# m-hamza-mughal/RAG-Gesture

Measured on AMD Instinct MI355X. Metric: SMPL-X frames/sec, len150 DDIM-50 + insertion guidance; 1/2/4/8 GPU, higher is better.
Workload: dtype bf16

## Files before the change

include/rg_gesture.h:

```cpp
#ifndef RG_GESTURE_H
#define RG_GESTURE_H

#include <stdint.h>

#ifdef __cplusplus
extern "C" {
#endif

typedef struct rg_handle rg_handle;

enum rg_status {
  RG_OK = 0,
  RG_ERR_INVALID = -1,
  RG_ERR_HIP = -2,
  RG_ERR_NO_DEVICE = -3
};

#define RG_VERSION 124
int rg_version(void);
int rg_create(rg_handle** out, int device);
void rg_destroy(rg_handle* h);
const char* rg_last_error(rg_handle* h);
int rg_num_cus(rg_handle* h);

int rg_ddim_update(rg_handle* h, const float* x, const float* x0, float* x_out, int64_t n,
                   float c_recip, float c_recipm1, float c_a, float c_b, void* stream);

int rg_cfg_ddim_update(rg_handle* h, const float* out, const float* x, float* x_out, float* x0_out,
                       const float* js, int B, int T, int D, float w_c, float w_u,
                       float c_recip, float c_recipm1, float c_a, float c_b, void* stream);
int rg_cfg_ddim_update_rows(rg_handle* h, const float* out_cond, const float* out_uncond, const float* x, float* x_out,
                            float* x_out2, const float* js, int B, int T, int D, float w_c, float w_u,
                            float c_recip, float c_recipm1, float c_a, float c_b, void* stream);

int rg_cfg_ddpm_update(rg_handle* h, const float* out, const float* x, const float* noise, float* x_out,
                       const float* js, int B, int T, int D, float w_c, float w_u, float c1, float c2, float sigma,
                       void* stream);

typedef struct rg_glue_args {
  const float* out_c_a;
  const float* out_u_a;
  float* x_a;
  const float* out_c_b;
  const float* out_u_b;
  float* x_b;
  float* x_b_copy;
  const float* in_seq_next;
  const float* noise_next;
  const float* js;
  int n_a, n_b, T, D;
  int g_iter_next;
// ... 139 lines not shown
#define RG_SEQ_U_FF2_0 12
#define RG_SEQ_U_FF1_1 13
#define RG_SEQ_U_FF2_1 14
#define RG_SEQ_U_FFO 15
typedef struct rg_seq_args {
  const void* wstream;
  const void* pstream;
  const void* ustream;
  const void* afrag;
  const float* x;
  const float* tbias;
  const float* src_mask;
  const float* qmask;
  float* head;
  float* dump;
  float* xbuf;
  void* gbuf;
  const int* form;
  int L, B, T, S;
  int step, step_b, split;
  int dump_stage, dump_layer;
  int pairs;
  int twin;
  int* glue_ctr;
  rg_glue_args glue;
} rg_seq_args;

int rg_seq_forward(rg_handle* h, const rg_seq_args* args_host, void* stream);
int rg_seq2_forward(rg_handle* h, const rg_seq_args* args_host, void* stream);

#define RG_SEQ_MANY_MAX 8
int rg_seq_forward_many(rg_handle* h, const rg_seq_args* const* args_host, int n, void* stream);

#define RG_LANE_STRIDE 32
int rg_seqx_forward(rg_handle* h, const rg_seq_args* args_host, void* stream);
int rg_lane_form(rg_handle* h, int* state, int lane, int nlanes, int narrow_wgs, int wide_wgs, int budget, void* stream);

typedef struct rg_venc_args {
  const void* wstream;
  const void* pstream;
  const float* x;
  float* out;
  float* xbuf;
  float* dump;
  int nseq, S, nb, dump_block;
  const int* post_rows;
  float* post_mu;
  float* post_logvar;
  int post_nrows, pad_;
} rg_venc_args;

int rg_venc_forward(rg_handle* h, const rg_venc_args* args_host, void* stream);
int rg_venc_forward_grouped(rg_handle* h, const rg_venc_args* args_host, int n, void* stream);

typedef struct rg_vdec_args {
  const void* wstream;
  const void* pstream;
  float* x;
  const float* pos;
  void* qimg;
  void* kbuf;
  void* vt;
  float* xbuf;
  float* dump;
  int nseq, nb, step, pad_;
  const float* latent;
// ... 419 lines not shown
```

rag-gesture_amd/csrc/rg_seq.hip:

```cpp
#ifndef RG_SEQ_BODY_ONLY
#define RG_PACK2_ONE
#endif
#include "rg_common.h"
#include "rg_stationary.h"
#include "rg_tail.h"
#include "rg_seq_host.h"

namespace {

constexpr int RD = 7;
constexpr int UPL = RG_SEQ_UPL;
constexpr int OFF_P0 = 0;
constexpr int OFF_P1 = TP * 1024;
constexpr int OFF_RING = 2 * TP * 1024;
constexpr int MAX_SEG = 8 * 34 + 5;
constexpr int OFF_DESC = OFF_RING + NW * RD * 1024;
constexpr int OFF_STAT = OFF_DESC + MAX_SEG * 16;
constexpr int LDS_BYTES = OFF_STAT + NW * TP * 2 * 4;
static_assert(LDS_BYTES <= 160 * 1024, "LDS budget");

#define U(name) U_##name = RG_SEQ_U_##name
enum { U(KV), U(KV2), U(Q), U(SAO), U(MIXX), U(Q3_0), U(MIX_0), U(Q3_1), U(MIX_1), U(Q3_2), U(MIX_2), U(FF1_0), U(FF2_0), U(FF1_1), U(FF2_1), U(FFO) };
#undef U
#define SEG(u, k) ((u) << 2 | (k))
// ... 491 lines not shown
  const int npass = pairs ? 2 : 1;
#pragma unroll 1
  for (int pass = 0; pass < npass; ++pass) {
    run_sequence(a, seq0 + pass * B, smem);
    __syncthreads();
    int* const ctr = rg_tail::late_ctr(arg_base);
    if (ctr && !a.dump_stage) {
      const int c = seq0 + pass * B - (seq0 + pass * B >= B ? B : 0);
      rg_tail::arrive_and_glue<NTH>(ctr, c, c, reinterpret_cast<int*>(smem), __builtin_amdgcn_readfirstlane(threadIdx.x >> 6), arg_base);
    }
  }
}

#ifndef RG_SEQ_BODY_ONLY
__global__ void __launch_bounds__(NTH) rg_seq_kernel(const rg_seq_args a) {
  extern __shared__ __attribute__((aligned(16))) unsigned char smem[];
  RG_OWN_THE_SIMD();
  seq_block(a, blockIdx.x, a.pairs, smem);
}

extern "C" int rg_seq_forward(rg_handle* h, const rg_seq_args* args_host, void* stream) {
  const std::string why = rg_seq_refusal(RG_SEQ_ENTRY, args_host);
  if (!why.empty()) { if (h) h->err = why; return RG_ERR_INVALID; }
  const rg_seq_args& a = *args_host;
  static rg_attr_once lds_once;
  RG_RESERVE_LDS(h, lds_once, rg_seq_kernel, LDS_BYTES);
  rg_prof_scope prof(h, stream, 3, rg_seq_flops(a));
  hipLaunchKernelGGL(rg_seq_kernel, dim3(a.pairs ? a.B : 2 * a.B), dim3(NTH), LDS_BYTES, rg_stream(stream), a);
  RG_CHECK_LAUNCH(h);
  prof.stop();
  return RG_OK;
}

struct rg_seq_many_block {
  rg_seq_args a[RG_SEQ_MANY_MAX];
  int end[RG_SEQ_MANY_MAX];
};
static_assert(sizeof(rg_seq_many_block) <= 4096, "the parameter block must fit the kernarg segment");

__global__ void __launch_bounds__(NTH) rg_seq_many_kernel(const rg_seq_many_block p) {
  extern __shared__ __attribute__((aligned(16))) unsigned char smem[];
  RG_OWN_THE_SIMD();
  const int block = blockIdx.x;
  int s = 0, first = 0;
#pragma unroll
  for (int i = 0; i + 1 < RG_SEQ_MANY_MAX; ++i)
    if (block >= p.end[i]) { s = i + 1; first = p.end[i]; }
  s = __builtin_amdgcn_readfirstlane(s);
  seq_block(p.a[s], block - first, 0, smem, (unsigned)(offsetof(rg_seq_many_block, a) + s * sizeof(rg_seq_args)));
}

extern "C" int rg_seq_forward_many(rg_handle* h, const rg_seq_args* const* args_host, int n, void* stream) {
  const std::string why = rg_seq_many_refusal(args_host, n);
  if (!why.empty()) { if (h) h->err = why; return RG_ERR_INVALID; }
  rg_seq_many_block p{};
  int total = 0;
  double flops = 0.0;
  for (int i = 0; i < RG_SEQ_MANY_MAX; ++i) {
    if (i < n) {
      p.a[i] = *args_host[i];
      total += 2 * p.a[i].B;
      flops += rg_seq_flops(p.a[i]);
    }
    p.end[i] = total;
  }
  static rg_attr_once lds_once;
  RG_RESERVE_LDS(h, lds_once, rg_seq_many_kernel, LDS_BYTES);
  rg_prof_scope prof(h, stream, 3, flops);
  hipLaunchKernelGGL(rg_seq_many_kernel, dim3(total), dim3(NTH), LDS_BYTES, rg_stream(stream), p);
  RG_CHECK_LAUNCH(h);
  prof.stop();
// ... 4 lines not shown
```

rag-gesture_amd/csrc/rg_seq2.hip:

```cpp
#if !defined(RG_SEQ_BODY_ONLY) && !defined(RG2_PACK_TWO)
#define RG_PACK2_ONE
#endif
#include "rg_common.h"
#include "rg_stationary.h"
#include "rg_tail.h"
#include "rg_seq_host.h"

namespace {

constexpr int RD = 6;
constexpr int UPL = RG_SEQ_UPL;
constexpr int PANEL = TP * 1024;
constexpr int OFF_RING = 2 * PANEL;
constexpr int NSEG_COND = 36, NSEG_UNC = 19, NSEG_TWIN = 34;
constexpr int NSEG_MAX = NSEG_COND > NSEG_TWIN ? NSEG_COND : NSEG_TWIN;
constexpr int MAX_SEG = 8 * NSEG_MAX + 5;
constexpr int OFF_DESC = OFF_RING + NW * RD * 1024;
constexpr int OFF_STAT = OFF_DESC + ((MAX_SEG * 8 + 15) & ~15);
constexpr int STAT_HALF = 2 * NW * TP * 2;
constexpr int LDS_BYTES = OFF_STAT + 2 * STAT_HALF * 4;
static_assert(LDS_BYTES <= 160 * 1024, "LDS budget");

#define U(name) U_##name = RG_SEQ_U_##name
enum { U(KV), U(KV2), U(Q), U(SAO), U(MIXX), U(Q3_0), U(MIX_0), U(Q3_1), U(MIX_1), U(Q3_2), U(MIX_2), U(FF1_0), U(FF2_0), U(FF1_1), U(FF2_1), U(FFO) };
// ... 925 lines not shown
__global__ void __launch_bounds__(NTH) rg_seq2_kernel(const rg_seq_args a) {
  extern __shared__ __attribute__((aligned(16))) unsigned char smem[];
#ifndef RG2_SHARE_SIMD
  RG_OWN_THE_SIMD();
#endif
  seq2_block(a, blockIdx.x, smem);
}

__global__ void __launch_bounds__(NTH) rg_seq2_twin_kernel(const rg_seq_args a) {
  extern __shared__ __attribute__((aligned(16))) unsigned char smem[];
#ifndef RG2_SHARE_SIMD
  RG_OWN_THE_SIMD();
#endif
  const int clip = blockIdx.x;
  run_pair<true>(a, clip, clip + a.B, smem);
  __syncthreads();
  if (rg_tail::late_ctr() && !a.dump_stage) rg_tail::glue_own<NTH>(clip, __builtin_amdgcn_readfirstlane(threadIdx.x >> 6));
}

extern "C" int rg_seq2_forward(rg_handle* h, const rg_seq_args* args_host, void* stream) {
  const std::string why = rg_seq_refusal(RG_SEQ2_ENTRY, args_host);
  if (!why.empty()) { if (h) h->err = why; return RG_ERR_INVALID; }
  const rg_seq_args& a = *args_host;
  static rg_attr_once lds_once, lds_once_twin;
  if (a.twin) { RG_RESERVE_LDS(h, lds_once_twin, rg_seq2_twin_kernel, LDS_BYTES); }
  else { RG_RESERVE_LDS(h, lds_once, rg_seq2_kernel, LDS_BYTES); }
  rg_prof_scope prof(h, stream, 3, rg_seq_flops(a));
  if (a.twin) hipLaunchKernelGGL(rg_seq2_twin_kernel, dim3(a.B), dim3(NTH), LDS_BYTES, rg_stream(stream), a);
  else hipLaunchKernelGGL(rg_seq2_kernel, dim3(seq2_grid(a.B, a.split, a.pairs)), dim3(NTH), LDS_BYTES, rg_stream(stream), a);
  RG_CHECK_LAUNCH(h);
  prof.stop();
  return RG_OK;
}
#endif
```

rag-gesture_amd/csrc/rg_seq_host.h:

```cpp
#pragma once
#include <string>

#include "../../include/rg_gesture.h"

struct rg_seq_entry { const char *name, *need_bufs, *need_form, *no_dump, *twin_range, *twin_pairs, *no_twin; };
constexpr rg_seq_entry RG_SEQ_ENTRY = {"rg_seq_forward", nullptr, nullptr, nullptr, nullptr, nullptr, nullptr};
constexpr rg_seq_entry RG_SEQ2_ENTRY = {"rg_seq2_forward", "the two-sequence forward needs its scratch buffers xbuf and gbuf", nullptr,
                                        nullptr, "twin must be 0 or 1", "twin and pairs are two launch forms: set one of them", nullptr};
constexpr rg_seq_entry RG_SEQX_ENTRY = {
    "rg_seqx_forward", "the two-sequence form needs its scratch buffers xbuf and gbuf", "form: the lane's flag (rg_lane_form) must be given",
    "diagnostic dumps: use rg_seq_forward / rg_seq2_forward", nullptr, nullptr,
    "the twin form (one clip per workgroup) is not one of the device-chosen forms: use rg_seq2_forward"};

inline bool rg_seq_glue_ok(const rg_seq_args& a) {
  if (!a.glue_ctr) return true;
  const rg_glue_args& g = a.glue;
  if (a.dump_stage || g.n_a < 0 || g.n_b < 0 || g.n_a + g.n_b != a.B || g.T != a.T || g.D != 512 || !g.js || g.g_iter_next < 0) return false;
  if (g.n_a && !(g.out_c_a && g.out_u_a && g.x_a)) return false;
  if (g.n_b && !(g.out_c_b && g.out_u_b && g.x_b)) return false;
  return !g.in_seq_next || g.noise_next;
}

inline std::string rg_seq_refusal(const rg_seq_entry& e, const rg_seq_args* args) {
  const char* why = nullptr;
// ... 6 lines not shown
    else if (e.need_form && !a.form) why = e.need_form;
    else if (!(a.L >= 1 && a.L <= 8 && a.B >= 1 && a.T >= 1 && a.T <= 48)) why = "unsupported shape (T <= 48, L <= 8)";
    else if (!(a.step >= 0 && a.step < a.S && a.step_b >= 0 && a.step_b < a.S)) why = "step out of range";
    else if (e.no_dump && a.dump_stage != 0) why = e.no_dump;
    else if (!e.no_dump && a.dump_stage != 0 && !a.dump) why = "dump_stage needs a dump buffer";
    else if (!(a.pairs == 0 || a.pairs == 1)) why = "pairs must be 0 or 1";
    else if (e.twin_range && !(a.twin == 0 || a.twin == 1)) why = e.twin_range;
    else if (e.twin_pairs && a.twin && a.pairs) why = e.twin_pairs;
    else if (e.no_twin && a.twin) why = e.no_twin;
    else if (!rg_seq_glue_ok(a)) why = "glue_ctr: glue must cover the B clips (n_a + n_b == B, T, D = 512), its pointers set, no dump";
  }
  return why ? std::string(e.name) + ": " + why : std::string();
}

constexpr rg_seq_entry RG_SEQ_MANY_ENTRY = {"rg_seq_forward_many", nullptr, nullptr, "diagnostic dumps: use rg_seq_forward", nullptr, nullptr,
                                            "the twin form is rg_seq2_forward's: a grouped launch runs one workgroup per sequence"};

inline std::string rg_seq_many_refusal(const rg_seq_args* const* args, const int n) {
  const std::string name = std::string(RG_SEQ_MANY_ENTRY.name) + ": ";
  if (!args || n < 1) return name + "null or empty list of sessions";
  if (n > RG_SEQ_MANY_MAX) return name + "too many sessions (at most RG_SEQ_MANY_MAX)";
  for (int i = 0; i < n; ++i) {
    const std::string why = rg_seq_refusal(RG_SEQ_MANY_ENTRY, args[i]);
    if (!why.empty()) return why;
    const rg_seq_args &a = *args[i], &a0 = *args[0];
    if (a.pairs) return name + "pairs is another launch form: a grouped launch runs one workgroup per sequence";
    if (!(a.L == a0.L && a.T == a0.T && a.S == a0.S)) return name + "the sessions must agree in L, T and S";
    if (!(a.wstream == a0.wstream && a.pstream == a0.pstream && a.ustream == a0.ustream))
      return name + "the sessions must share the weight, parameter and table streams";
  }
  return std::string();
}

inline double rg_seq_flops(const rg_seq_args& a) {
  const double unit = 2.0 * a.T * 512 * 512, att = 2.0 * a.T * 32 * 32 * 16;
  const double cond = (RG_SEQ_UPL * a.L + 2) * unit + a.L * (2 + 3) * att, unc = (10 * a.L + 2) * unit + a.L * 2 * att;
  return a.B * (cond + unc);
}
```

rag-gesture_amd/csrc/rg_tail.h:

```cpp
#pragma once
#include "rg_common.h"
#include <cstddef>

namespace rg_tail {

typedef __attribute__((ext_vector_type(4))) float f32x4;
typedef __attribute__((ext_vector_type(4))) unsigned u32x4;
constexpr int COHERENT = 17;

__device__ __forceinline__ float ddim_one(float x, float x0, float c_recip, float c_recipm1, float c_a, float c_b) {
#pragma clang fp contract(off)
  float eps = (c_recip * x - x0) / c_recipm1;
  return x0 * c_a + c_b * eps;
}
__device__ __forceinline__ float cfg_one(float oc, float ou, float jc, float ju, float w_c, float w_u) {
#pragma clang fp contract(off)
  return oc * w_c * jc + ou * w_u * ju;
}

template <typename P>
__device__ __forceinline__ P* uniform_ptr(P* p) {
  const unsigned long long v = reinterpret_cast<unsigned long long>(p);
  return reinterpret_cast<P*>((unsigned long long)__builtin_amdgcn_readfirstlane((unsigned)(v >> 32)) << 32 |
                              (unsigned)__builtin_amdgcn_readfirstlane((unsigned)v));
// ... 143 lines not shown

__device__ __forceinline__ void store_head(float* head, const unsigned byte_offset, const f32x4 v) {
  const auto rs = __builtin_amdgcn_make_buffer_rsrc(head, 0, 0x7fffffff, 0x00020000);
  __builtin_amdgcn_raw_buffer_store_b128(__builtin_bit_cast(u32x4, v), rs, byte_offset, 0, COHERENT);
}

template <int NTH>
__device__ __forceinline__ void arrive_and_glue(int* const ctr, const int c0, const int c1, int* const flag, const int wave,
                                                const unsigned base = 0) {
  const int lane = __builtin_amdgcn_mbcnt_hi(~0u, __builtin_amdgcn_mbcnt_lo(~0u, 0u));
  if (wave == 0 && lane == 0) {
    int m = 0;
    if (__hip_atomic_fetch_add(ctr + c0, 1, __ATOMIC_RELAXED, __HIP_MEMORY_SCOPE_AGENT) & 1) m |= 1;
    if (c1 != c0 && (__hip_atomic_fetch_add(ctr + c1, 1, __ATOMIC_RELAXED, __HIP_MEMORY_SCOPE_AGENT) & 1)) m |= 2;
    *flag = m;
  }
  __syncthreads();
  const int m = *flag;
  __syncthreads();
  if (m == 0) return;
  const rg_glue_args g = late_arg<rg_glue_args>(base + offsetof(rg_seq_args, glue));
  const float ton = two_over_numel(g);
#pragma unroll 1
  for (int q = 0; q < 2; ++q) {
    if (!(m >> q & 1)) continue;
    const int c = q ? c1 : c0;
    const bool ga = c < g.n_a;
    const int cl = ga ? c : c - g.n_a;
    glue_clip<NTH / 64>(g, ga, cl, wave, lane, ton);
  }
}

template <int NTH>
__device__ __forceinline__ void glue_own(const int c, const int wave) {
  const int lane = __builtin_amdgcn_mbcnt_hi(~0u, __builtin_amdgcn_mbcnt_lo(~0u, 0u));
  const rg_glue_args g = late_arg<rg_glue_args>(offsetof(rg_seq_args, glue));
  const bool ga = c < g.n_a;
  glue_clip<NTH / 64>(g, ga, ga ? c : c - g.n_a, wave, lane, two_over_numel(g));
}
}
```

rag-gesture_amd/denoiser.py:

```python
import math

import numpy as np
import torch

from . import capi, gemm as G, seqfwd as SQ

CONDS = ("xf_text", "xf_audio", "xf_spk")
BLOCKS = ("sa_block", "ca_blocks.xf_text", "ca_blocks.xf_audio", "ca_blocks.xf_spk", "ffn")


def _timestep_embedding(timesteps, dim, max_period=10000):
    half = dim // 2
    freqs = torch.exp(-math.log(max_period) * torch.arange(0, half, dtype=torch.float32) / half)
    args = timesteps[:, None].float() * freqs[None]
    return torch.cat([torch.cos(args), torch.sin(args)], dim=-1)


class DenoiserWeights:

    KV_GROUP = 2

    @staticmethod
    def _fold_ln(W, b, gamma, beta, pw, f32):
        Wp = (W.double() * gamma.double()[None, :]).float()
# ... 316 lines not shown
        key = (name, tuple(shape), dtype)
        pool = self.__dict__.setdefault("_scratch_pool", {})
        if key not in pool:
            pool[key] = torch.empty(*shape, device=self.w.dev, dtype=dtype)
        return pool[key]

    def chain_end(self):
        if self.sq is not None:
            self.sq.chain_end()

    def forward(self, x, step, step_b=None, split=None, glue=None):
        w, h, B, R, M, D, T = self.w, self.h, self.B, self.R, self.M, self.w.D, self.w.T
        if split is not None and not (0 < split < B):
            step, step_b, split = (step if split >= B else step_b), None, None
        if self.sq is not None:
            if glue is not None and not x.is_contiguous():
                raise capi.RgError("DenoiserSession.forward(glue=...): x is updated in place and must be contiguous")
            return self.sq.run(x.contiguous(), step, step_b, split, glue=glue)
        if glue is not None:
            raise capi.RgError("DenoiserSession.forward(glue=...): the sequence-stationary engine only")
        if self.ln_mode == "auto":
            out = self._forward_guarded(x, step)
            if split is None:
                return out
        return self._forward_chain(x, step, step_b, split)

    @staticmethod
    def forward_many(sessions, calls):
        for s, kw in zip(sessions, calls):
            if s.sq is None or not kw["x"].is_contiguous():
                raise capi.RgError("DenoiserSession.forward_many: the sequence-stationary engine only, x contiguous")
        return SQ.run_many([s.sq for s in sessions], calls)

    LN_GUARD_SIGMAS = 3.0

    def _forward_guarded(self, x, step):
        if torch.cuda.is_current_stream_capturing():
            raise capi.RgError("DenoiserSession(ln_mode='auto'): run one forward before capturing a graph")
        self._guard = torch.zeros(1, device=self.w.dev)
        self.ln_mode = "folded"
        out = self._forward_chain(x, step)
        self.ln_ratio = float(self._guard.item())
        self._guard = None
        if self.ln_ratio > self.LN_GUARD_SIGMAS ** 2:
            self.ln_mode, self.xa_bf = "prologue", None
            out = self._forward_chain(x, step)
        return out

    def _guard_stats(self, stats):
        if getattr(self, "_guard", None) is not None:
            self.h.call("ln_guard", stats, self.M, stats.shape[1], self.w.D, self._guard)

    def _forward_chain(self, x, step, step_b=None, split=None):
        w, h, B, R, M, D, T = self.w, self.h, self.B, self.R, self.M, self.w.D, self.w.T
        two = split is not None
        if two and (self.abf is None or self.hcat is None):
            raise capi.RgError("two step groups: bf16 launch chain with the stylization pre-pass only")
        xa, xb, xc = self.xa, self.xb, self.xc
        sa_, sb_, sc_ = self.st_a, self.st_b, self.st_c
        sa_w = self.st_a
        G.gemm(h, M=M, N=D, K=D, W=w.w_embed, out=xa, segs=[G.Seg(x.view(B * T, D))], seg_len=D, a_row_mod=B * T,
               bias=w.b_embed, tbias=w.tbias, tb_period=T, stats_out=sa_, out2=self.xa_bf)
        self._guard_stats(sa_)
        for l, lw in enumerate(w.layers):
            ss = w.ss[step, l]
            ssb = w.ss[step_b, l] if two else None
# ... 104 lines not shown
```

rag-gesture_amd/pipeline.py:

```python
import collections
import ctypes
import contextlib
import copy
import os
import time
import types

import torch
import yaml

from . import capi, denoiser, sampler, schedule as sched_mod, seqfwd, vae as vae_mod

MODELS = {}


def register_module(cls):
    MODELS[cls.__name__] = cls
    return cls


def register_with_mmcv(force=False):
    regs = []
    try:
        from mmcv.cnn import MODELS as mmcv_models
# ... 244 lines not shown
        return dict.__iter__(self)

    def copy(self):
        self._ready()
        return dict(dict.items(self))

    __copy__ = copy

    def __deepcopy__(self, memo):
        self._ready()
        return {k: copy.deepcopy(v, memo) for k, v in dict.items(self) if k not in self._PLAIN}

    def __reduce__(self):
        self._ready()
        return (dict, (), None, None, iter([(k, v) for k, v in dict.items(self) if k not in self._PLAIN]))


@register_module
class MotionDiffusion(torch.nn.Module):

    profile_phases = False
    rotation_lanes = None
    form_lanes = None
    _cur_rot = None
    _last_state = None

    def __init__(self, model=None, loss_recon=None, loss_gen=None, loss_contact=None, loss_laplace=None,
                 diffusion_train=None, diffusion_test=None, init_cfg=None, inference_type="ddpm",
                 genloss_acceleration_weight=True, genloss_hands_weight=2, genloss_smooth=True,
                 body_part_lossweights=None, device="cuda", precision="bf16", lanes=2, sample_lanes=None, session_options=None,
                 vae_options=None, async_results=False, slots=2, max_inflight=2, cobatch_lanes="batch", base_lanes=8,
                 batch_lanes=4, lane_streams=None, calibrate_lanes=True, decode_stream=False, dynamic_forms=False, dynamic_budget=None, invert_alone_wide=True, tail_glue=True,
                 cache_exemplar_latents=True, exemplar_cache_bytes=8 << 30, skip_clip_encode=True, grouped_decode=True,
                 grouped_drain=True, **kwargs):
        super().__init__()
        self.grouped_drain = bool(grouped_drain)
        self.grouped_decode = bool(grouped_decode)
        self.cache_exemplar_latents, self.exemplar_cache_bytes = bool(cache_exemplar_latents), int(exemplar_cache_bytes)
        self.skip_clip_encode = bool(skip_clip_encode)
        self.model = build_submodule(model, device=device, **kwargs)
        dt = dict(diffusion_test)
        self.schedule = sched_mod.Schedule(beta_scheduler=dt["beta_scheduler"], diffusion_steps=dt["diffusion_steps"],
                                           respace=dt.get("respace"))
        capi.require(dt.get("model_mean_type", "start_x") == "start_x" and dt.get("classifier_free_guidance_scale", 0) == 0,
                "unsupported argument: requires dt.get(\"model_mean_type\", \"start_x\") == \"start_x\" and dt.get(\"classifier_free_guidance_scale\", 0) == 0")
        self.inference_type = inference_type
        capi.require(inference_type in ("ddim", "ddpm"), "inference_type is 'ddim' (shipped config) or 'ddpm'")
        self.device, self.precision = torch.device(device), precision
        self.training = False
        self.session_options, self.vae_options = dict(session_options or {}), dict(vae_options or {})
        self.vae_options.setdefault("grouped_decode", self.grouped_decode)
        self._state = None
        self._sessions = {}
        self._graphs = {}
        self.use_graphs = True
        self.graph_captures = self.graph_cross_stream_waits = 0
        self._jitter = None
        self.phase_ms = {}
        self.lanes = int(lanes)
        self.base_lanes = max(1, int(base_lanes))
        self.batch_lanes = max(1, int(batch_lanes))
        self.sample_lanes = None if sample_lanes is None else int(sample_lanes)
        self.async_results, self.slots, self.max_inflight = bool(async_results), max(1, int(slots)), max(1, int(max_inflight))
        self.dynamic_forms, self._lane_state = bool(dynamic_forms), None
        self.invert_alone_wide = bool(invert_alone_wide)
        self.tail_glue = bool(tail_glue)
        self.dynamic_budget = None if dynamic_budget is None else int(dynamic_budget)
        self._slot, self._inflight, self._graph_owner, self._slot_done = 0, collections.deque(), {}, {}
# ... 491 lines not shown
            h = self.model.weights.h
            for idx in st.idx_groups:
                h.call("copy_rows", lat.contiguous(), st.in_seq, st.B, 1, st.D, st.T, idx[-1], st.T, idx[0])

    def _take_slot(self, pid, main, lanes, slot=None):
        slot = self._slots[pid] = (self._slots.get(pid, 0) + 1) % self.slots if slot is None else slot
        self._wait_slot(main, lanes, slot)
        self._slot = slot
        return slot

    def _wait_slot(self, main, lanes, slot):
        for lane in dict.fromkeys(lanes):
            for ev in self._slot_done.get((lane, slot), ()):
                main.wait_event(ev)

    @staticmethod
    def _lanes_of(*plans):
        return list(dict.fromkeys(lane for plan in plans for lane, _, _, _ in plan))

    def submit(self, **kwargs):
        if not self.async_results or self.slots < 2:
            raise capi.RgError("submit() needs MotionDiffusion(async_results=True, slots >= 2)")
        self._cob = dict(lane=self._submitted if (self.cobatch_lanes == "batch" and self.batch_lanes > 1) else None)
        self._submitted += 1
        try:
            self.forward(**kwargs)
        finally:
            self._cob = None
        return self._ready.popleft() if self._ready else None

    def flush(self):
        cob, self._cob = self._cob, dict(lane=0)
        try:
            self._finish_pending()
        finally:
            self._cob = cob
        out = list(self._ready)
        self._ready.clear()
        return out

    def _finish_alone(self, st):
        main = st.main = torch.cuda.current_stream()
        st.slot = self._take_slot(st.pid, main, self._lanes_of(st.plan_s))
        for lane, stream, b0, b1 in st.plan_s:
            self._sample_conditions(lane, b0, b1, st.word, st.audio, st.spk, st.motion_mask, st.qmask)
        self._sampling_pass(st)
        return self._tail(st)

    def _pending_upto(self, seq):
        return sorted((p for p in self._pend if self._pend[p].seq <= seq), key=lambda p: self._pend[p].seq)

    def _finish_pending(self, upto=None, resume=None):
        sts = [self._pend.pop(p) for p in self._pending_upto(float("inf") if upto is None else upto)]
        group = self._drain_group(sts) if self.grouped_drain else []
        if group:
            self._drain_grouped(group)
        for st in sts:
            self._ready.append(self._tail(st) if any(st is g for g in group) else self._finish_alone(st))
        if resume is not None:
            self._slot = self._slots[resume.pid] = resume.slot

    DRAIN_SLOT = 0

    def _drain_group(self, sts):
        sett = lambda st: (st.T, st.S, bool(st.use_insertion_guidance), tuple(int(v) for v in st.guidance_iters), float(st.guidance_lr))

        def alone_on_a_lane(st):
            return (st.run_async and st.via_submit and not st.ddpm and st.prev_future is None and st.plan == st.plan_s
                    and len(st.plan_s) == 1 and tuple(st.plan_s[0][2:]) == (0, st.B))
# ... 43 lines not shown
        owners = tuple((st.B, "sample", st.plan_s[0][0], st.slot) for st in order)
        key = ("guided_many" if guided else "sample_many", owners, order[0].T, tuple(st.in_seq is not None for st in order), gi, lr)
        with torch.cuda.stream(g), self._phase("sampling"):
            outs = self._graph_run(key, ins, loop, owner=owners)
            for st, xl in zip(order, outs):
                st.x_out.copy_(xl)

    def _set_conditions_pair(self, sess, key, own, a, b, n_a):
        dev = self.model.weights.dev
        ins = {}
        for tag, (word, audio, spk, mask, qm) in (("a", a), ("b", b)):
            ins["word_" + tag], ins["audio_" + tag] = word.to(dev).float(), audio.to(dev).float()
            ins["spk_" + tag], ins["mask_" + tag] = spk.to(dev).long(), mask.to(dev).float()
            for c in denoiser.CONDS:
                ins["q_%s_%s" % (c, tag)] = qm[c].to(dev).float()

        def run(st):
            for tag, off, fin in (("a", 0, False), ("b", n_a, True)):
                sess.set_conditions(st["word_" + tag], st["audio_" + tag], st["spk_" + tag], st["mask_" + tag],
                                    {c: st["q_%s_%s" % (c, tag)] for c in denoiser.CONDS}, offset=off, finalize=fin)
            return ()
        self._graph_run(key + tuple(tuple(v.shape) for v in ins.values()), ins, run, owner=own)

    def _submit_chain(self, st):
        pend, S, T, D, dev = self._pend.get(st.pid), st.S, st.T, st.D, self.device
        lanes = [(lane, stream, b0, b1, self._exemplars(st, b0, b1)) for lane, stream, b0, b1 in st.plan] if st.use_inversion else []
        so = self.session_options
        groups_ok = self.precision == "bf16" and (self._runs_seq_engine(so) or so.get("styl_prepass", True))
        can_defer = (groups_ok and st.use_inversion and not st.visualize_inversion and not st.ddpm and st.plan == st.plan_s
                     and all(ex for *_, ex in lanes))
        same = pend is not None and can_defer and (pend.B, pend.T) == (st.B, st.T) and \
            [(b0, b1) for _, _, b0, b1 in pend.plan] == [(b0, b1) for _, _, b0, b1 in st.plan]
        if pend is not None and not same:
            self._finish_pending(pend.seq, resume=st)
            pend = None
        if not can_defer:
            self._finish_pending(resume=st)
            for lane, stream, b0, b1 in st.plan_s:
                self._sample_conditions(lane, b0, b1, st.word, st.audio, st.spk, st.motion_mask, st.qmask)
            self._inversion_pass(st)
            self._sampling_pass(st)
            self._ready.append(self._tail(st))
            return None
        if pend is None:
            self._inversion_pass(st)
            for lane, stream, _, _ in st.plan:
                self._slot_done[(lane, st.slot)] = [stream.record_event()]
            self._pend[st.pid] = st
            return None
        main = st.main
        self._fill_prev(pend, main)
        guided = pend.use_insertion_guidance
        gi, lr = tuple(int(v) for v in pend.guidance_iters), float(pend.guidance_lr)
        work = []
        for lane, stream, b0, b1, ex in lanes:
            Bl = b1 - b0
            Ep, cat = self._exemplar_inputs(st, ex, main)
            okey = (Bl + Ep, "cobatch", lane, self._slot)
            sess = self._session(Bl + Ep, "cobatch", lane)
            eqm = exemplar_query_masks(st.qmask, [b for b, _ in ex], Ep)
            self._set_conditions_pair(
                sess, ("cond2", Bl, Ep, lane, self._slot), okey,
                (pend.word[b0:b1], pend.audio[b0:b1], pend.spk[b0:b1], pend.motion_mask[b0:b1], {c: pend.qmask[b0:b1] for c in denoiser.CONDS}),
                (cat("retr_text"), cat("retr_audio"), cat("retr_spkid"), cat("retr_motion_mask"), eqm), Bl)
            work.append((lane, stream, b0, b1, ex, Ep, sess, okey, cat("retr_motion_latent").float().contiguous()))
        for lane, stream, b0, b1, ex, Ep, sess, okey, x_e in work:
            Bl = b1 - b0
            stream.wait_stream(main)
            self._used_on(stream, pend.x, pend.in_seq, pend.inseq_noise, pend.invl, pend.x_out, x_e, st.start_noise, st.invl, st.qmask)
            with torch.cuda.stream(stream):
                sl = lambda t, dim: lane_rows(t, dim, b0, b1)
                ins = dict(xa=sl(pend.x, 0), in_seq=sl(pend.in_seq, 0), noise=sl(pend.inseq_noise, 1),
                           invl=sl(pend.invl, 1) if guided else None, xb=x_e)

                def loop(s, sess=sess, Bl=Bl, Ep=Ep):
                    x_all = torch.cat([s["xa"], s["xb"]], dim=0).contiguous()
                    out_b = torch.empty(S, Ep, T, D, device=dev)
                    sampler.cobatched_loop(sess, x_all, Bl, out_b, inverted_a=s["invl"], guidance_iters=gi, guidance_lr=lr,
                                           inseq_noise_a=s["noise"], in_seq_a=s["in_seq"], tail_glue=self.tail_glue)
                    return x_all[:Bl], out_b
                key = ("cobatch", Bl, Ep, lane, T, self._slot, guided, pend.in_seq is not None, gi, lr, self.tail_glue)
                xl, inv = self._graph_run(key, ins, loop, owner=okey)
                pend.x_out[b0:b1].copy_(xl)
                self._splice(st, ex, inv, Ep)
                self._zero_prev_rows(st, b0, b1)
        pend.main, pend.slot = main, self._slot
        self._ready.append(self._tail(pend))
        self._pend[st.pid] = st
        return None

    def _exemplars(self, st, b0, b1):
        return [(b, q) for b in range(b0, b1) for q in st.retrieval_dict["retr_uncropped_latents"][b].keys()]

    def _exemplar_inputs(self, st, ex, stream):
        dev = self.device
        Ep = bucket(len(ex))
        lat = lambda b, q: st.retrieval_dict["retr_uncropped_latents"][b][q]

        def cat(key):
            parts = [lat(b, q)[key].to(dev) for b, q in ex]
            self._used_on(stream, *parts)
            return pad_rows(torch.cat(parts, dim=0), Ep)
        return Ep, cat

    def _splice(self, st, ex, inv, Ep):
        h, rd = self.model.weights.h, st.retrieval_dict
        lvl = st.inversion_start_time % st.S
        rows = []
        for e, (b, q_idx) in enumerate(ex):
            r0, r1 = rd["retr_startends"][b][q_idx]
            q0, q1 = rd["query_startends"][b][q_idx]
            capi.require(r1 - r0 == q1 - q0, "unsupported argument: requires r1 - r0 == q1 - q0")
            rows.append((e, b, int(r0), int(q0), int(r1 - r0)))
        invl = st.invl if st.use_insertion_guidance else None
        capi.require(inv.is_contiguous() and st.start_noise.is_contiguous() and (invl is None or invl.is_contiguous()),
                     "splice: contiguous tensors expected")
        for c0 in range(0, len(rows), sampler.SPLICE_MAX):
            tab = sampler.SpliceTable()
            chunk = rows[c0:c0 + sampler.SPLICE_MAX]
            tab.n = len(chunk)
            for i, (e, b, r0, q0, n) in enumerate(chunk):
                tab.e[i], tab.b[i], tab.r0[i], tab.q0[i], tab.nrows[i] = e, b, r0, q0, n
# ... 126 lines not shown
```

rag-gesture_amd/sampler.py:

```python
import ctypes

import torch

from . import capi

from .seqfwd import GlueArgs, MANY_MAX

SPLICE_MAX = capi.header_constants()["RG_SPLICE_MAX"]
SpliceTable = capi.struct("rg_splice_table")


TAIL_GLUE = True


def _tail_ok(sess, x):
    return (TAIL_GLUE and getattr(sess, "tail_glue", True) and getattr(sess, "sq", None) is not None and sess.h.recorder is None and x.is_cuda and x.is_contiguous()
            and x.dtype == torch.float32 and x.shape[0] == sess.B)


def _p(t):
    if t is None:
        return None
    if not (t.is_cuda and t.is_contiguous() and t.dtype == torch.float32):
        raise capi.RgError("rg_cobatch_glue: contiguous fp32 device tensors expected")
# ... 128 lines not shown


def cobatched_loop(sess, x_all, n_a, out_b, inverted_a=None, guidance_iters=None, guidance_lr=0.1, inseq_noise_a=None,
                   in_seq_a=None, fused_glue=True, tail_glue=True):
    h, S, B = sess.h, sess.w.schedule.num_timesteps, sess.B
    n_b = B - n_a
    xa, xb = x_all[:n_a], x_all[n_a:]
    in_seq = in_seq_a
    if fused_glue and h.recorder is None:
        _insert_first(sess, xa, n_a, in_seq, inseq_noise_a)
        tail = bool(tail_glue) and _tail_ok(sess, x_all) and 0 < n_a < B
        for k in range(S):
            i = S - 1 - k
            if not tail:
                sess.forward(x_all, i, step_b=k, split=n_a)
            nxt = None if i == 0 else (inverted_a[i - 1] if inverted_a is not None else in_seq_a)
            a = _glue(sess, guidance_lr, i=i, x_a=xa, n_a=n_a, nxt=nxt, noise_nxt=None if nxt is None else inseq_noise_a[i - 1],
                      g_next=guidance_iters[i - 1] if inverted_a is not None and i > 0 else 0, k=k, x_b=xb, keep_b=out_b[k], n_b=n_b)
            if tail:
                sess.forward(x_all, i, step_b=k, split=n_a, glue=a)
            else:
                h.call("cobatch_glue", ctypes.byref(a))
        sess.chain_end()
        return x_all, out_b
    for k in range(S):
        i, g_iter = S - 1 - k, None
        if inverted_a is not None and i != S - 1:
            in_seq, g_iter = inverted_a[i], guidance_iters[i]
        _step(sess, xa, i, in_seq, None if in_seq is None else inseq_noise_a[i], g_iter, guidance_lr, n_a, (x_all, k, xb, out_b[k]))
    sess.chain_end()
    return x_all, out_b


class GraphedLoop:

    def __init__(self, fn, warmup=True):
        if warmup:
            s = torch.cuda.Stream()
            s.wait_stream(torch.cuda.current_stream())
            with torch.cuda.stream(s):
                fn()
            torch.cuda.current_stream().wait_stream(s)
        self.graph = torch.cuda.CUDAGraph()
        with capi.capture(self.graph):
            fn()

    def replay(self):
        self.graph.replay()
```

rag-gesture_amd/seqfwd.py:

```python
import ctypes

import torch

from . import capi

_C = capi.header_constants()
UPL = _C["RG_SEQ_UPL"]
(U_KV, U_KV2, U_Q, U_SAO, U_MIXX, U_Q3_0, U_MIX_0, U_Q3_1, U_MIX_1, U_Q3_2, U_MIX_2, U_FF1_0, U_FF2_0, U_FF1_1, U_FF2_1, U_FFO) = (
    _C["RG_SEQ_U_" + n] for n in "KV KV2 Q SAO MIXX Q3_0 MIX_0 Q3_1 MIX_1 Q3_2 MIX_2 FF1_0 FF2_0 FF1_1 FF2_1 FFO".split())
CONDS = ("xf_text", "xf_audio", "xf_spk")
LANE_STRIDE = _C["RG_LANE_STRIDE"]
GlueArgs = capi.struct("rg_glue_args")
SeqArgs = capi.struct("rg_seq_args")


def supported(cfg, T, precision):
    return (precision == "bf16" and cfg["latent_dim"] == 512 and cfg["num_heads"] == 16 and cfg["ff_size"] == 1024
            and T <= 48 and 1 <= cfg["num_layers"] <= 8)


def pack_unit(W):
    capi.require(W.shape == (512, 512), "unsupported argument: requires W.shape == (512, 512)")
    v = W.to(torch.bfloat16).view(8, 4, 16, 16, 4, 8)
    return v.permute(0, 3, 1, 4, 2, 5).contiguous().view(8, 64, 64, 8)
# ... 134 lines not shown
            if glue.n_a + glue.n_b != self.sess.B or glue.T != self.sess.w.T or glue.D != self.sess.w.D or dump_stage:
                raise capi.RgError("rg_seq_forward: the tail's groups must cover the session's clips (n_a + n_b == B)")
            a.glue, a.glue_ctr = glue, self.glue_ctr.data_ptr()
        else:
            a.glue_ctr = None
        if not (x.is_contiguous() and x.dtype == torch.float32 and x.numel() == self.sess.B * self.sess.w.T * self.sess.w.D):
            raise capi.RgError("rg_seq_forward: x must be a contiguous fp32 [B, T, D] tensor")
        a.x, a.step = x.data_ptr(), int(step)
        a.step_b = int(step if step_b is None else step_b)
        a.split = int(self.sess.B if split is None else split)
        a.dump = dump.data_ptr() if dump is not None else None
        a.dump_stage, a.dump_layer = int(dump_stage), int(dump_layer)
        return a

    def run(self, x, step, step_b=None, split=None, dump=None, dump_stage=0, dump_layer=0, glue=None):
        a = self._set_args(x, step, step_b, split, dump, dump_stage, dump_layer, glue)
        if self.lane_dyn is not None and not dump_stage:
            state, lane, n, budget = self.lane_dyn
            B = self.sess.B
            wide = 2 * B
            if self.duo:
                sp = max(0, min(B, a.split))
                npc = (sp + 1) // 2 + (B - sp + 1) // 2
                narrow = npc if a.pairs else 2 * npc
            else:
                narrow = wide = B if a.pairs else 2 * B
            self.h.call("lane_form", state, lane, n, narrow, wide, budget)
        self.h.call("seq2_forward" if dump_stage and self.lane_dyn is not None and self.duo else self._entry, ctypes.byref(a))
        return self.sess.head

    def groupable(self):
        return not self.duo and not self.twin and not self.args.pairs and self.lane_dyn is None

    def chain_end(self):
        if self.lane_dyn is not None:
            state, lane, n, budget = self.lane_dyn
            self.h.call("lane_form", state, lane, n, 0, 0, budget)


MANY_MAX = _C["RG_SEQ_MANY_MAX"]


def run_many(sqs, calls):
    if not (1 <= len(sqs) <= MANY_MAX and len(sqs) == len(calls)):
        raise capi.RgError("rg_seq_forward_many: 1 to %d sessions, one set of arguments each" % MANY_MAX)
    if not all(sq.groupable() for sq in sqs):
        raise capi.RgError("rg_seq_forward_many: sessions in the one-workgroup-per-sequence form only (no duo, pairs, twin or lane_dyn)")
    args = [sq._set_args(**kw) for sq, kw in zip(sqs, calls)]
    ptrs = (ctypes.c_void_p * len(args))(*[ctypes.addressof(a) for a in args])
    sqs[0].h.call("seq_forward_many", ctypes.cast(ptrs, ctypes.c_void_p), len(args))
    return [sq.sess.head for sq in sqs]
```

Before: 70480.

## Group held cobatch requests into one multi-session twin kernel launch per step

```diff
diff --git a/include/rg_gesture.h b/include/rg_gesture.h
--- a/include/rg_gesture.h
+++ b/include/rg_gesture.h
@@ -16,7 +16,7 @@
   RG_ERR_NO_DEVICE = -3
 };
 
-#define RG_VERSION 124
+#define RG_VERSION 125
 int rg_version(void);
 int rg_create(rg_handle** out, int device);
 void rg_destroy(rg_handle* h);
@@ -222,6 +222,8 @@
 #define RG_SEQ_MANY_MAX 8
 int rg_seq_forward_many(rg_handle* h, const rg_seq_args* const* args_host, int n, void* stream);
 
+int rg_seq2_twin_forward_many(rg_handle* h, const rg_seq_args* const* args_host, int n, void* stream);
+
 #define RG_LANE_STRIDE 32
 int rg_seqx_forward(rg_handle* h, const rg_seq_args* args_host, void* stream);
 int rg_lane_form(rg_handle* h, int* state, int lane, int nlanes, int narrow_wgs, int wide_wgs, int budget, void* stream);
diff --git a/rag-gesture_amd/csrc/rg_seq.hip b/rag-gesture_amd/csrc/rg_seq.hip
--- a/rag-gesture_amd/csrc/rg_seq.hip
+++ b/rag-gesture_amd/csrc/rg_seq.hip
@@ -547,11 +547,6 @@
   return RG_OK;
 }
 
-struct rg_seq_many_block {
-  rg_seq_args a[RG_SEQ_MANY_MAX];
-  int end[RG_SEQ_MANY_MAX];
-};
-static_assert(sizeof(rg_seq_many_block) <= 4096, "the parameter block must fit the kernarg segment");
 
 __global__ void __launch_bounds__(NTH) rg_seq_many_kernel(const rg_seq_many_block p) {
   extern __shared__ __attribute__((aligned(16))) unsigned char smem[];
diff --git a/rag-gesture_amd/csrc/rg_seq2.hip b/rag-gesture_amd/csrc/rg_seq2.hip
--- a/rag-gesture_amd/csrc/rg_seq2.hip
+++ b/rag-gesture_amd/csrc/rg_seq2.hip
@@ -981,4 +981,49 @@
   prof.stop();
   return RG_OK;
 }
+
+__global__ void __launch_bounds__(NTH) rg_seq2_twin_many_kernel(const rg_seq_many_block p) {
+  extern __shared__ __attribute__((aligned(16))) unsigned char smem[];
+#ifndef RG2_SHARE_SIMD
+  RG_OWN_THE_SIMD();
 #endif
+  const int block = blockIdx.x;
+  int s = 0, first = 0;
+#pragma unroll
+  for (int i = 0; i + 1 < RG_SEQ_MANY_MAX; ++i)
+    if (block >= p.end[i]) { s = i + 1; first = p.end[i]; }
+  s = __builtin_amdgcn_readfirstlane(s);
+  const unsigned base = (unsigned)(offsetof(rg_seq_many_block, a) + s * sizeof(rg_seq_args));
+  const rg_seq_args& a = p.a[s];
+  const int clip = block - first;
+  run_pair<true>(a, clip, clip + a.B, smem);
+  __syncthreads();
+  if (rg_tail::late_ctr(base) && !a.dump_stage) rg_tail::glue_own<NTH>(clip, __builtin_amdgcn_readfirstlane(threadIdx.x >> 6), base);
+}
+
+extern "C" int rg_seq2_twin_forward_many(rg_handle* h, const rg_seq_args* const* args_host, int n, void* stream) {
+  const std::string why = rg_seq2_twin_many_refusal(args_host, n);
+  if (!why.empty()) { if (h) h->err = why; return RG_ERR_INVALID; }
+  rg_seq_many_block p{};
+  int total = 0;
+  double flops = 0.0;
+  for (int i = 0; i < RG_SEQ_MANY_MAX; ++i) {
+    if (i < n) {
+      rg_seq_args& a = p.a[i];
+      a = *args_host[i];
+      a.xbuf = reinterpret_cast<float*>(reinterpret_cast<uintptr_t>(a.xbuf) - (uintptr_t)total * (2 * NW * 12 * 64 * 4 * sizeof(float)));
+      a.gbuf = reinterpret_cast<void*>(reinterpret_cast<uintptr_t>(a.gbuf) - (uintptr_t)total * (8 * PANEL));
+      total += a.B;
+      flops += rg_seq_flops(a);
+    }
+    p.end[i] = total;
+  }
+  static rg_attr_once lds_once;
+  RG_RESERVE_LDS(h, lds_once, rg_seq2_twin_many_kernel, LDS_BYTES);
+  rg_prof_scope prof(h, stream, 3, flops);
+  hipLaunchKernelGGL(rg_seq2_twin_many_kernel, dim3(total), dim3(NTH), LDS_BYTES, rg_stream(stream), p);
+  RG_CHECK_LAUNCH(h);
+  prof.stop();
+  return RG_OK;
+}
+#endif
diff --git a/rag-gesture_amd/csrc/rg_seq_host.h b/rag-gesture_amd/csrc/rg_seq_host.h
--- a/rag-gesture_amd/csrc/rg_seq_host.h
+++ b/rag-gesture_amd/csrc/rg_seq_host.h
@@ -62,6 +62,33 @@
   return std::string();
 }
 
+struct rg_seq_many_block {
+  rg_seq_args a[RG_SEQ_MANY_MAX];
+  int end[RG_SEQ_MANY_MAX];
+};
+static_assert(sizeof(rg_seq_many_block) <= 4096, "the parameter block must fit the kernarg segment");
+
+constexpr rg_seq_entry RG_SEQ2_TWIN_MANY_ENTRY = {
+    "rg_seq2_twin_forward_many", "the two-sequence forward needs its scratch buffers xbuf and gbuf", nullptr,
+    "diagnostic dumps: use rg_seq2_forward", "twin must be 0 or 1", "twin and pairs are two launch forms: set one of them", nullptr};
+
+inline std::string rg_seq2_twin_many_refusal(const rg_seq_args* const* args, const int n) {
+  const std::string name = std::string(RG_SEQ2_TWIN_MANY_ENTRY.name) + ": ";
+  if (!args || n < 1) return name + "null or empty list of sessions";
+  if (n > RG_SEQ_MANY_MAX) return name + "too many sessions (at most RG_SEQ_MANY_MAX)";
+  for (int i = 0; i < n; ++i) {
+    const std::string why = rg_seq_refusal(RG_SEQ2_TWIN_MANY_ENTRY, args[i]);
+    if (!why.empty()) return why;
+    const rg_seq_args &a = *args[i], &a0 = *args[0];
+    if (a.pairs) return name + "pairs is another launch form: a grouped twin launch runs one workgroup per clip";
+    if (!a.twin) return name + "every session must be in the twin form (twin == 1): the other forms are rg_seq2_forward's and rg_seq_forward_many's";
+    if (!(a.L == a0.L && a.T == a0.T && a.S == a0.S)) return name + "the sessions must agree in L, T and S";
+    if (!(a.wstream == a0.wstream && a.pstream == a0.pstream && a.ustream == a0.ustream))
+      return name + "the sessions must share the weight, parameter and table streams";
+  }
+  return std::string();
+}
+
 inline double rg_seq_flops(const rg_seq_args& a) {
   const double unit = 2.0 * a.T * 512 * 512, att = 2.0 * a.T * 32 * 32 * 16;
   const double cond = (RG_SEQ_UPL * a.L + 2) * unit + a.L * (2 + 3) * att, unc = (10 * a.L + 2) * unit + a.L * 2 * att;
diff --git a/rag-gesture_amd/csrc/rg_tail.h b/rag-gesture_amd/csrc/rg_tail.h
--- a/rag-gesture_amd/csrc/rg_tail.h
+++ b/rag-gesture_amd/csrc/rg_tail.h
@@ -199,9 +199,9 @@
 }
 
 template <int NTH>
-__device__ __forceinline__ void glue_own(const int c, const int wave) {
+__device__ __forceinline__ void glue_own(const int c, const int wave, const unsigned base = 0) {
   const int lane = __builtin_amdgcn_mbcnt_hi(~0u, __builtin_amdgcn_mbcnt_lo(~0u, 0u));
-  const rg_glue_args g = late_arg<rg_glue_args>(offsetof(rg_seq_args, glue));
+  const rg_glue_args g = late_arg<rg_glue_args>(base + offsetof(rg_seq_args, glue));
   const bool ga = c < g.n_a;
   glue_clip<NTH / 64>(g, ga, ga ? c : c - g.n_a, wave, lane, two_over_numel(g));
 }
diff --git a/rag-gesture_amd/denoiser.py b/rag-gesture_amd/denoiser.py
--- a/rag-gesture_amd/denoiser.py
+++ b/rag-gesture_amd/denoiser.py
@@ -372,6 +372,13 @@
                 raise capi.RgError("DenoiserSession.forward_many: the sequence-stationary engine only, x contiguous")
         return SQ.run_many([s.sq for s in sessions], calls)
 
+    @staticmethod
+    def forward_twin_many(sessions, calls):
+        for s, kw in zip(sessions, calls):
+            if s.sq is None or not kw["x"].is_contiguous():
+                raise capi.RgError("DenoiserSession.forward_twin_many: the sequence-stationary engine only, x contiguous")
+        return SQ.run_twin_many([s.sq for s in sessions], calls)
+
     LN_GUARD_SIGMAS = 3.0
 
     def _forward_guarded(self, x, step):
diff --git a/rag-gesture_amd/pipeline.py b/rag-gesture_amd/pipeline.py
--- a/rag-gesture_amd/pipeline.py
+++ b/rag-gesture_amd/pipeline.py
@@ -300,8 +300,9 @@
                  vae_options=None, async_results=False, slots=2, max_inflight=2, cobatch_lanes="batch", base_lanes=8,
                  batch_lanes=4, lane_streams=None, calibrate_lanes=True, decode_stream=False, dynamic_forms=False, dynamic_budget=None, invert_alone_wide=True, tail_glue=True,
                  cache_exemplar_latents=True, exemplar_cache_bytes=8 << 30, skip_clip_encode=True, grouped_decode=True,
-                 grouped_drain=True, **kwargs):
+                 grouped_drain=True, cobatch_group=2, **kwargs):
         super().__init__()
+        self.cobatch_group, self._held, self._held_any = max(1, int(cobatch_group)), [], False
         self.grouped_drain = bool(grouped_drain)
         self.grouped_decode = bool(grouped_decode)
         self.cache_exemplar_latents, self.exemplar_cache_bytes = bool(cache_exemplar_latents), int(exemplar_cache_bytes)
@@ -859,9 +860,13 @@
     def flush(self):
         cob, self._cob = self._cob, dict(lane=0)
         try:
+            self._release_held()
             self._finish_pending()
         finally:
             self._cob = cob
+        if self._held_any:
+            self._slots.clear()
+            self._held_any = False
         out = list(self._ready)
         self._ready.clear()
         return out
@@ -971,9 +976,11 @@
         same = pend is not None and can_defer and (pend.B, pend.T) == (st.B, st.T) and \
             [(b0, b1) for _, _, b0, b1 in pend.plan] == [(b0, b1) for _, _, b0, b1 in st.plan]
         if pend is not None and not same:
+            self._release_held(resume=st)
             self._finish_pending(pend.seq, resume=st)
             pend = None
         if not can_defer:
+            self._release_held(resume=st)
             self._finish_pending(resume=st)
             for lane, stream, b0, b1 in st.plan_s:
                 self._sample_conditions(lane, b0, b1, st.word, st.audio, st.spk, st.motion_mask, st.qmask)
@@ -988,9 +995,12 @@
             self._pend[st.pid] = st
             return None
         main = st.main
+        hold = self._can_hold(st, pend, lanes)
+        if not hold or any(c.st is pend for c in self._held) or (self._held and self._hold_sett(pend) != self._hold_sett(self._held[0].pend)):
+            self._release_held(resume=st)
+        if hold:
+            st.slot = self._take_slot(st.pid, main, [lanes[0][0]], slot=(st.seq // self._rotation()) % self.slots)
         self._fill_prev(pend, main)
-        guided = pend.use_insertion_guidance
-        gi, lr = tuple(int(v) for v in pend.guidance_iters), float(pend.guidance_lr)
         work = []
         for lane, stream, b0, b1, ex in lanes:
             Bl = b1 - b0
@@ -1002,31 +1012,119 @@
                 sess, ("cond2", Bl, Ep, lane, self._slot), okey,
                 (pend.word[b0:b1], pend.audio[b0:b1], pend.spk[b0:b1], pend.motion_mask[b0:b1], {c: pend.qmask[b0:b1] for c in denoiser.CONDS}),
                 (cat("retr_text"), cat("retr_audio"), cat("retr_spkid"), cat("retr_motion_mask"), eqm), Bl)
-            work.append((lane, stream, b0, b1, ex, Ep, sess, okey, cat("retr_motion_latent").float().contiguous()))
-        for lane, stream, b0, b1, ex, Ep, sess, okey, x_e in work:
-            Bl = b1 - b0
-            stream.wait_stream(main)
-            self._used_on(stream, pend.x, pend.in_seq, pend.inseq_noise, pend.invl, pend.x_out, x_e, st.start_noise, st.invl, st.qmask)
-            with torch.cuda.stream(stream):
-                sl = lambda t, dim: lane_rows(t, dim, b0, b1)
-                ins = dict(xa=sl(pend.x, 0), in_seq=sl(pend.in_seq, 0), noise=sl(pend.inseq_noise, 1),
-                           invl=sl(pend.invl, 1) if guided else None, xb=x_e)
-
-                def loop(s, sess=sess, Bl=Bl, Ep=Ep):
-                    x_all = torch.cat([s["xa"], s["xb"]], dim=0).contiguous()
-                    out_b = torch.empty(S, Ep, T, D, device=dev)
-                    sampler.cobatched_loop(sess, x_all, Bl, out_b, inverted_a=s["invl"], guidance_iters=gi, guidance_lr=lr,
-                                           inseq_noise_a=s["noise"], in_seq_a=s["in_seq"], tail_glue=self.tail_glue)
-                    return x_all[:Bl], out_b
-                key = ("cobatch", Bl, Ep, lane, T, self._slot, guided, pend.in_seq is not None, gi, lr, self.tail_glue)
-                xl, inv = self._graph_run(key, ins, loop, owner=okey)
-                pend.x_out[b0:b1].copy_(xl)
-                self._splice(st, ex, inv, Ep)
-                self._zero_prev_rows(st, b0, b1)
+            work.append(types.SimpleNamespace(
+                st=st, pend=pend, main=main, lane=lane, stream=stream, b0=b0, b1=b1, ex=ex, Ep=Ep, sess=sess, okey=okey,
+                x_e=cat("retr_motion_latent").float().contiguous(), slot=self._slot, cur_rot=self._cur_rot))
+        self._pend[st.pid] = st
+        if hold:
+            self._held.append(work[0])
+            self._held_any = True
+            if len(self._held) >= min(self.cobatch_group, self._rotation()):
+                self._release_held(resume=st)
+            return None
+        for c in work:
+            self._chain_alone(c)
         pend.main, pend.slot = main, self._slot
         self._ready.append(self._tail(pend))
-        self._pend[st.pid] = st
         return None
+
+    def _rotation(self):
+        return max(1, min(int(self.rotation_lanes or self.batch_lanes), max(1, len(self._lane_streams))))
+
+    @staticmethod
+    def _hold_sett(pend):
+        return (pend.T, pend.S, bool(pend.use_insertion_guidance), tuple(int(v) for v in pend.guidance_iters), float(pend.guidance_lr))
+
+    def _can_hold(self, st, pend, lanes):
+        if not (self.cobatch_group > 1 and self.precision == "bf16" and self._rotation() > 1 and st.pid is not None and len(lanes) == 1
+                and st.run_async and st.via_submit and pend.prev_future is None and st.prev_future is None):
+            return False
+        lane, _, b0, b1, ex = lanes[0]
+        o = self._session_opts(b1 - b0 + bucket(len(ex)), "cobatch", lane)
+        return bool((b0, b1) == (0, st.B) and self._runs_seq_engine(o) and o["seq_twin"] and o.get("seq_duo") and not o.get("seq_pairs")
+                    and "lane_dyn" not in o and o["tail_glue"] and self.tail_glue and sampler.TAIL_GLUE
+                    and self.model.weights.h.recorder is None)
+
+    def _chain_alone(self, c):
+        st, pend, b0, b1, Ep, sess = c.st, c.pend, c.b0, c.b1, c.Ep, c.sess
+        S, T, D, dev, Bl = st.S, st.T, st.D, self.device, c.b1 - c.b0
+        guided = pend.use_insertion_guidance
+        gi, lr = tuple(int(v) for v in pend.guidance_iters), float(pend.guidance_lr)
+        c.stream.wait_stream(c.main)
+        self._used_on(c.stream, pend.x, pend.in_seq, pend.inseq_noise, pend.invl, pend.x_out, c.x_e, st.start_noise, st.invl, st.qmask)
+        with torch.cuda.stream(c.stream):
+            sl = lambda t, dim: lane_rows(t, dim, b0, b1)
+            ins = dict(xa=sl(pend.x, 0), in_seq=sl(pend.in_seq, 0), noise=sl(pend.inseq_noise, 1),
+                       invl=sl(pend.invl, 1) if guided else None, xb=c.x_e)
+
+            def loop(s):
+                x_all = torch.cat([s["xa"], s["xb"]], dim=0).contiguous()
+                out_b = torch.empty(S, Ep, T, D, device=dev)
+                sampler.cobatched_loop(sess, x_all, Bl, out_b, inverted_a=s["invl"], guidance_iters=gi, guidance_lr=lr,
+                                       inseq_noise_a=s["noise"], in_seq_a=s["in_seq"], tail_glue=self.tail_glue)
+                return x_all[:Bl], out_b
+            key = ("cobatch", Bl, Ep, c.lane, T, c.slot, guided, pend.in_seq is not None, gi, lr, self.tail_glue)
+            xl, inv = self._graph_run(key, ins, loop, owner=c.okey)
+            pend.x_out[b0:b1].copy_(xl)
+            self._splice(st, c.ex, inv, Ep)
+            self._zero_prev_rows(st, b0, b1)
+
+    def _release_held(self, resume=None):
+        held, self._held = self._held, []
+        if not held:
+            return
+        slot, rot = self._slot, self._cur_rot
+        self._slot, self._cur_rot = held[0].slot, held[0].cur_rot
+        try:
+            if len(held) == 1:
+                self._chain_alone(held[0])
+            else:
+                self._launch_held_group(held)
+            for c in held:
+                c.pend.main, c.pend.slot = c.main, c.slot
+                self._ready.append(self._tail(c.pend))
+        finally:
+            self._slot, self._cur_rot = (resume.slot if resume is not None else slot), rot
+
+    def _launch_held_group(self, held):
+        order = sorted(held, key=lambda c: c.lane)
+        n, g, p0 = len(order), order[0].stream, order[0].pend
+        S, T, D, dev = p0.S, p0.T, p0.D, self.device
+        guided = bool(p0.use_insertion_guidance)
+        gi, lr = tuple(int(v) for v in p0.guidance_iters), float(p0.guidance_lr)
+        ins = {}
+        for k, c in enumerate(order):
+            st, pend = c.st, c.pend
+            g.wait_stream(c.main)
+            if c.stream is not g:
+                g.wait_stream(c.stream)
+            self._used_on(g, pend.x, pend.in_seq, pend.inseq_noise, pend.invl, pend.x_out, c.x_e, st.start_noise, st.invl, st.qmask)
+            ins.update({"xa%d" % k: pend.x, "in_seq%d" % k: pend.in_seq, "noise%d" % k: pend.inseq_noise,
+                        "invl%d" % k: pend.invl if guided else None, "xb%d" % k: c.x_e})
+        sessions, n_as, eps = [c.sess for c in order], [c.b1 - c.b0 for c in order], [c.Ep for c in order]
+
+        def loop(s):
+            x_alls = [torch.cat([s["xa%d" % k], s["xb%d" % k]], dim=0).contiguous() for k in range(n)]
+            out_bs = [torch.empty(S, eps[k], T, D, device=dev) for k in range(n)]
+            col = lambda name: [s["%s%d" % (name, k)] for k in range(n)]
+            sampler.cobatched_loop_many(sessions, x_alls, n_as, out_bs, inverted_as=col("invl"), guidance_iters=gi, guidance_lr=lr,
+                                        inseq_noise_as=col("noise"), in_seq_as=col("in_seq"), tail_glue=self.tail_glue)
+            return tuple(t for k in range(n) for t in (x_alls[k][:n_as[k]], out_bs[k]))
+        owners = tuple(c.okey for c in order)
+        key = ("cobatch_many", tuple((c.b1 - c.b0, c.Ep, c.lane, c.slot) for c in order), T, guided,
+               tuple(c.pend.in_seq is not None for c in order), gi, lr, self.tail_glue)
+        with torch.cuda.stream(g), self._phase("sampling"):
+            outs = self._graph_run(key, ins, loop, owner=owners)
+            res = {id(c): (outs[2 * k], outs[2 * k + 1]) for k, c in enumerate(order)}
+            for c in held:
+                xl, inv = res[id(c)]
+                c.pend.x_out[c.b0:c.b1].copy_(xl)
+                self._splice(c.st, c.ex, inv, c.Ep)
+                self._zero_prev_rows(c.st, c.b0, c.b1)
+        for c in order:
+            if c.stream is not g:
+                c.stream.wait_stream(g)
+            c.pend.wait_streams = [g]
 
     def _exemplars(self, st, b0, b1):
         return [(b, q) for b in range(b0, b1) for q in st.retrieval_dict["retr_uncropped_latents"][b].keys()]
diff --git a/rag-gesture_amd/sampler.py b/rag-gesture_amd/sampler.py
--- a/rag-gesture_amd/sampler.py
+++ b/rag-gesture_amd/sampler.py
@@ -184,6 +184,41 @@
     return x_all, out_b
 
 
+def twin_many_ok(sessions, x_alls, n_as, tail_glue=True):
+    return (bool(tail_glue) and 1 < len(sessions) <= MANY_MAX
+            and all(_tail_ok(s, x) and s.sq.twin_groupable() and 0 < n < s.B for s, x, n in zip(sessions, x_alls, n_as))
+            and all(s.w is sessions[0].w for s in sessions) and len({id(s) for s in sessions}) == len(sessions))
+
+
+def cobatched_loop_many(sessions, x_alls, n_as, out_bs, inverted_as=None, guidance_iters=None, guidance_lr=0.1, inseq_noise_as=None,
+                        in_seq_as=None, tail_glue=True):
+    n = len(sessions)
+    none = [None] * n
+    inverted_as, inseq_noise_as, in_seq_as = (none if v is None else v for v in (inverted_as, inseq_noise_as, in_seq_as))
+    if not twin_many_ok(sessions, x_alls, n_as, tail_glue):
+        for k in range(n):
+            cobatched_loop(sessions[k], x_alls[k], n_as[k], out_bs[k], inverted_a=inverted_as[k], guidance_iters=guidance_iters,
+                           guidance_lr=guidance_lr, inseq_noise_a=inseq_noise_as[k], in_seq_a=in_seq_as[k], tail_glue=tail_glue)
+        return x_alls, out_bs
+    S = sessions[0].w.schedule.num_timesteps
+    for k, sess in enumerate(sessions):
+        _insert_first(sess, x_alls[k][:n_as[k]], n_as[k], in_seq_as[k], inseq_noise_as[k])
+    for j in range(S):
+        i = S - 1 - j
+        calls = []
+        for k, sess in enumerate(sessions):
+            n_a = n_as[k]
+            nxt = None if i == 0 else (inverted_as[k][i - 1] if inverted_as[k] is not None else in_seq_as[k])
+            calls.append(dict(x=x_alls[k], step=i, step_b=j, split=n_a, glue=_glue(
+                sess, guidance_lr, i=i, x_a=x_alls[k][:n_a], n_a=n_a, nxt=nxt, noise_nxt=None if nxt is None else inseq_noise_as[k][i - 1],
+                g_next=guidance_iters[i - 1] if inverted_as[k] is not None and i > 0 else 0,
+                k=j, x_b=x_alls[k][n_a:], keep_b=out_bs[k][j], n_b=sess.B - n_a)))
+        type(sessions[0]).forward_twin_many(sessions, calls)
+    for sess in sessions:
+        sess.chain_end()
+    return x_alls, out_bs
+
+
 class GraphedLoop:
 
     def __init__(self, fn, warmup=True):
diff --git a/rag-gesture_amd/seqfwd.py b/rag-gesture_amd/seqfwd.py
--- a/rag-gesture_amd/seqfwd.py
+++ b/rag-gesture_amd/seqfwd.py
@@ -190,6 +190,9 @@
     def groupable(self):
         return not self.duo and not self.twin and not self.args.pairs and self.lane_dyn is None
 
+    def twin_groupable(self):
+        return self.duo and self.twin and not self.args.pairs and self.lane_dyn is None
+
     def chain_end(self):
         if self.lane_dyn is not None:
             state, lane, n, budget = self.lane_dyn
@@ -208,3 +211,14 @@
     ptrs = (ctypes.c_void_p * len(args))(*[ctypes.addressof(a) for a in args])
     sqs[0].h.call("seq_forward_many", ctypes.cast(ptrs, ctypes.c_void_p), len(args))
     return [sq.sess.head for sq in sqs]
+
+
+def run_twin_many(sqs, calls):
+    if not (1 <= len(sqs) <= MANY_MAX and len(sqs) == len(calls)):
+        raise capi.RgError("rg_seq2_twin_forward_many: 1 to %d sessions, one set of arguments each" % MANY_MAX)
+    if not all(sq.twin_groupable() for sq in sqs):
+        raise capi.RgError("rg_seq2_twin_forward_many: sessions in the twin form only (duo and twin, no pairs or lane_dyn)")
+    args = [sq._set_args(**kw) for sq, kw in zip(sqs, calls)]
+    ptrs = (ctypes.c_void_p * len(args))(*[ctypes.addressof(a) for a in args])
+    sqs[0].h.call("seq2_twin_forward_many", ctypes.cast(ptrs, ctypes.c_void_p), len(args))
+    return [sq.sess.head for sq in sqs]
```

Result: no change. 70640, median of 2 (+0.2%).
